# lixirui142/VidToMe

Measured on AMD Instinct MI355X. Metric: denoising steps/sec, 16-frame 512x512 SD-1.5 chunk, ratio=0.5, higher is better.
Workload: dtype f16 tokens; matching f16-MFMA filter + f32 exact refine (f32-identical indices); attention f16 MFMA with f32 accumulate

## Files before the change

### include/vidtome_hip.h

```cpp
#ifndef VIDTOME_HIP_H
#define VIDTOME_HIP_H

#include <stddef.h>
#include <stdint.h>

#ifdef __cplusplus
extern "C" {
#endif

#define VTM_ABI_VERSION 2

enum vtm_dtype { VTM_F32 = 0, VTM_F16 = 1, VTM_BF16 = 2 };

enum vtm_status {
    VTM_OK = 0,
    VTM_EINVAL = -1,
    VTM_ELAUNCH = -2,
    VTM_EWORKSPACE = -3
};

typedef void *vtm_stream_t;

int vtm_version(void);
const char *vtm_last_error(void);
// ... 12 lines not shown
              int64_t Nd_pad, int64_t C_pad, int align, uint64_t *best, vtm_stream_t stream);

size_t vtm_match_filtered_ws_bytes(int64_t B, int64_t C, int64_t Ns, int64_t Nd, int align);
int vtm_match_filtered(const void *x0, int64_t P0, const void *x1, int64_t P1, int dtype, int64_t B,
                       int64_t C, const int32_t *a_rows, int64_t Ns, const int32_t *b_rows, int64_t Nd,
                       int align, void *ws, size_t ws_bytes, uint64_t *best, int32_t *flags_out,
                       vtm_stream_t stream);
int vtm_match_filtered_seeded(const void *x0, int64_t P0, const void *x1, int64_t P1, int dtype, int64_t B,
                              int64_t C, const int32_t *a_rows, int64_t Ns, const int32_t *b_rows, int64_t Nd,
                              int align, void *ws, size_t ws_bytes, uint64_t *best, int32_t *flags_out,
                              int64_t seed_L, int64_t seed_N, const int32_t *seed_pos1, const int32_t *seed_table,
                              vtm_stream_t stream);
#define VTM_MATCH_ONE_LAUNCH 0
#define VTM_MATCH_SCOUT_RANGE 1
#define VTM_MATCH_SCOUT_STEPS(k) (((k) & 0xff) << 8)
int vtm_match_filtered_plan(const void *x0, int64_t P0, const void *x1, int64_t P1, int dtype, int64_t B,
                            int64_t C, const int32_t *a_rows, int64_t Ns, const int32_t *b_rows, int64_t Nd,
                            int align, void *ws, size_t ws_bytes, uint64_t *best, int32_t *flags_out,
                            int64_t seed_L, int64_t seed_N, const int32_t *seed_pos1, const int32_t *seed_table,
                            int mode, vtm_stream_t stream);

#define VTM_POSITION_ORDER_MAX_N 16360
size_t vtm_position_order_counter_ints(int64_t B, int64_t N);
size_t vtm_position_order_ws_bytes(int64_t B, int64_t Ns, int64_t Nd, int64_t N);
int vtm_position_order(const int32_t *a_rows, int64_t Ns, const int32_t *b_rows, int64_t Nd, int64_t B, int64_t L,
                       int64_t N, const int32_t *pos1, int64_t P0, int64_t P1, int32_t *counters, void *ws,
                       size_t ws_bytes, int32_t *a_sorted, int32_t *a_order, int32_t *b_sorted, int32_t *b_order,
                       int32_t *table, int shared_order, vtm_stream_t stream);
int vtm_match_filtered_ordered(const void *x0, int64_t P0, const void *x1, int64_t P1, int dtype, int64_t B,
                               int64_t C, const int32_t *a_sorted, int64_t Ns, const int32_t *b_sorted, int64_t Nd,
                               int align, void *ws, size_t ws_bytes, uint64_t *best, int32_t *flags_out, int64_t seed_L,
                               int64_t seed_N, const int32_t *seed_pos1, const int32_t *seed_table, int mode,
                               const int32_t *a_order, const int32_t *b_order, vtm_stream_t stream);

int vtm_decode_best(const uint64_t *best, int64_t n, float *node_max, int32_t *node_idx,
// ... 158 lines not shown
```

### vidtome_amd/_lib.py

```python
from __future__ import annotations

import ctypes
import functools
import os
import threading
from typing import Optional, Tuple

import torch

_HERE = os.path.dirname(os.path.abspath(__file__))
ABI_VERSION = 2
LIB_PATH = os.environ.get("VIDTOME_HIP_LIB") or os.path.join(_HERE, "lib", "libvidtome_hip.so")

VTM_F32, VTM_F16, VTM_BF16 = 0, 1, 2
ROW_PAD, K_PAD = 256, 32

_DT = {torch.float32: VTM_F32, torch.float16: VTM_F16, torch.bfloat16: VTM_BF16}

_vp, _i64, _int, _f32 = ctypes.c_void_p, ctypes.c_int64, ctypes.c_int, ctypes.c_float
_lib: Optional[ctypes.CDLL] = None

_SIGNATURES = {
    "vtm_version": ([], _int),
    "vtm_last_error": ([], ctypes.c_char_p),
    "vtm_build_ablations": ([], _int),
    "vtm_pad_rows": ([_i64], _i64),
    "vtm_pad_k": ([_i64], _i64),
    "vtm_normalize_gather": ([_vp, _i64, _vp, _i64, _int, _i64, _i64, _vp, _i64, _vp, _vp, _i64, _i64, _vp], _int),
    "vtm_match": ([_vp, _vp, _i64, _i64, _i64, _i64, _i64, _i64, _int, _vp, _vp], _int),
    "vtm_match_filtered_ws_bytes": ([_i64, _i64, _i64, _i64, _int], ctypes.c_size_t),
    "vtm_match_filtered": ([_vp, _i64, _vp, _i64, _int, _i64, _i64, _vp, _i64, _vp, _i64, _int, _vp, ctypes.c_size_t,
                            _vp, _vp, _vp], _int),
    "vtm_match_filtered_plan": ([_vp, _i64, _vp, _i64, _int, _i64, _i64, _vp, _i64, _vp, _i64, _int, _vp, ctypes.c_size_t,
                                 _vp, _vp, _i64, _i64, _vp, _vp, _int, _vp], _int),
    "vtm_match_filtered_ordered": ([_vp, _i64, _vp, _i64, _int, _i64, _i64, _vp, _i64, _vp, _i64, _int, _vp, ctypes.c_size_t,
                                    _vp, _vp, _i64, _i64, _vp, _vp, _int, _vp, _vp, _vp], _int),
    "vtm_position_order_counter_ints": ([_i64, _i64], ctypes.c_size_t),
    "vtm_position_order_ws_bytes": ([_i64, _i64, _i64, _i64], ctypes.c_size_t),
    "vtm_position_order": ([_vp, _i64, _vp, _i64, _i64, _i64, _i64, _vp, _i64, _i64, _vp, _vp, ctypes.c_size_t, _vp, _vp, _vp,
                            _vp, _vp, _int, _vp], _int),
    "vtm_match_filtered_seeded": ([_vp, _i64, _vp, _i64, _int, _i64, _i64, _vp, _i64, _vp, _i64, _int, _vp, ctypes.c_size_t,
                                   _vp, _vp, _i64, _i64, _vp, _vp, _vp], _int),
    "vtm_anchor_pos": ([_vp, _i64, _i64, _i64, _i64, _vp, _i64, _vp, _vp], _int),
    "vtm_decode_best": ([_vp, _i64, _vp, _vp, _vp], _int),
    "vtm_sort_ws_bytes": ([_i64, _i64], ctypes.c_size_t),
    "vtm_sort_desc": ([_vp, _i64, _i64, _vp, _vp, ctypes.c_size_t, _vp], _int),
    "vtm_partition_counts": ([_i64, _i64, _i64, _i64, _i64, ctypes.POINTER(_i64), ctypes.POINTER(_i64)], _int),
    "vtm_partition_local": ([_vp, _i64, _i64, _i64, _i64, _i64, _i64, _vp, _vp, _vp, _vp, _i64, _i64, _vp], _int),
    "vtm_partition_global": ([_vp, _i64, _i64, _i64, _i64, _int, _vp, _vp, _vp, _vp, _vp, _i64, _vp, _vp], _int),
    "vtm_plan_apply": ([_vp, _vp, _vp, _vp, _vp, _vp, _i64, _i64, _i64, _i64, _i64, _int, _vp, _vp, _vp, _vp,
                        _vp, _vp], _int),
# ... 163 lines not shown
                                      _ptr(norms), _ptr(out), n_pad, C_pad, _stream()), "vtm_normalize_gather")
    return out, norms


@_on_device
def match(a: torch.Tensor, b: torch.Tensor, Ns: int, Nd: int, align: bool) -> torch.Tensor:
    B, G, _, Ns_pad, _ = a.shape
    C_pad, Nd_pad = G * 8, b.shape[3]
    best = torch.empty((1 if align else B, Ns), dtype=torch.int64, device=a.device)
    _check(lib().vtm_match(_ptr(a), _ptr(b), B, Ns, Nd, Ns_pad, Nd_pad, C_pad, int(align), _ptr(best), _stream()),
           "vtm_match")
    return best


MATCH_ONE_LAUNCH, MATCH_SCOUT_RANGE = 0, 1


@_on_device
def match_filtered(x0: torch.Tensor, x1: Optional[torch.Tensor], a_rows: torch.Tensor, b_rows: torch.Tensor,
                   align: bool, want_flag: bool = False, seed=None, mode: int = MATCH_ONE_LAUNCH,
                   stats_host: Optional[torch.Tensor] = None, order=None, scout_steps: int = 0):
    _req(x0, "x0"), _req(a_rows, "a_rows"), _req(b_rows, "b_rows")
    B, P0, C = x0.shape
    P1 = 0 if x1 is None else _req(x1, "x1").shape[1]
    Ns, Nd = a_rows.shape[1], b_rows.shape[1]
    nbytes = lib().vtm_match_filtered_ws_bytes(B, C, Ns, Nd, int(align))
    ws = _workspace("match", nbytes, x0.device)
    best = torch.empty((1 if align else B, Ns), dtype=torch.int64, device=x0.device)
    flag = torch.zeros((8,), dtype=torch.int32, device=x0.device) if want_flag else None
    flags_out = _ptr(flag)
    if flag is None and stats_host is not None:
        if not (stats_host.is_pinned() and stats_host.dtype == torch.int32 and stats_host.numel() >= 8):
            raise RuntimeError("match_filtered: stats_host must be a pinned int32 tensor of 8 elements")
        flags_out = stats_host.data_ptr()
    mode = int(mode) | ((int(scout_steps) & 0xff) << 8)
    sN = sL = 0
    pos1 = table = None
    if seed is not None and SEED_MATCHER:
        sN, sL, pos1, table = seed
        if pos1 is not None and (pos1.dtype != torch.int32 or tuple(pos1.shape) != (B, P1) or not pos1.is_contiguous()):
            raise RuntimeError("match_filtered: seed positions must be a contiguous (B, P1) int32 tensor")
        if table is not None and (table.dtype != torch.int32 or tuple(table.shape) != (B, sN) or not table.is_contiguous()):
            raise RuntimeError("match_filtered: the seed table must be a contiguous (B, N) int32 tensor")
    if order is not None:
        a_order, b_order = order
        for o, n, name in ((a_order, Ns, "a_order"), (b_order, Nd, "b_order")):
            if o.dtype != torch.int32 or tuple(o.shape) != (B, n) or not o.is_contiguous() or not o.is_cuda:
                raise RuntimeError(f"match_filtered: {name} must be a contiguous (B, {n}) int32 device tensor")
        _check(lib().vtm_match_filtered_ordered(_ptr(x0), P0, _ptr(x1), P1, dtype_code(x0), B, C, _ptr(a_rows), Ns,
                                                _ptr(b_rows), Nd, int(align), _ptr(ws), nbytes, _ptr(best), flags_out, int(sL), int(sN),
                                                _ptr(pos1), _ptr(table), int(mode), _ptr(a_order), _ptr(b_order), _stream()),
               "vtm_match_filtered_ordered")
        return (best, flag) if want_flag else best
    _check(lib().vtm_match_filtered_plan(_ptr(x0), P0, _ptr(x1), P1, dtype_code(x0), B, C, _ptr(a_rows), Ns,
                                         _ptr(b_rows), Nd, int(align), _ptr(ws), nbytes, _ptr(best), flags_out,
                                         int(sL), int(sN), _ptr(pos1), _ptr(table), int(mode), _stream()),
           "vtm_match_filtered_plan")
    return (best, flag) if want_flag else best


POSITION_ORDER_MAX_N = 16360
_ZEROED: dict = {}


def _zeroed_counters(n_ints: int, device: torch.device) -> torch.Tensor:
    key = (device.index, torch.cuda.current_stream(device).cuda_stream, threading.get_ident())
    buf = _ZEROED.get(key)
    if buf is None or buf.numel() < n_ints:
        buf = torch.zeros((max(int(n_ints), 16),), dtype=torch.int32, device=device)
        with _WS_LOCK:
            _ZEROED[key] = buf
    return buf

# ... 715 lines not shown
```

### vidtome_amd/csrc/match_filter.hip

```cpp
#include "common.h"
#include "ablate.h"
#include "match_plan.h"

#include <algorithm>
#include <type_traits>

namespace {

using namespace vtm_match_plan;
static_assert(MODE_SCOUT_RANGE == VTM_MATCH_SCOUT_RANGE, "match_plan.h restates the public mode value");
constexpr int THREADS = 256;
constexpr float SCALE = 1024.0f;
constexpr float INV_S2 = 1.0f / (1024.0f * 1024.0f);
constexpr float WINDOW = SRC_LO ? 6.5e-4f : DST_LO ? 1.5e-3f : 2.4e-3f;
constexpr int MAX_C = 1280;

typedef float f32x16 __attribute__((ext_vector_type(16)));
typedef _Float16 h16x8 __attribute__((ext_vector_type(8)));
typedef uint32_t u32x4 __attribute__((ext_vector_type(4)));
typedef __attribute__((address_space(3))) void lds_void;
typedef const __attribute__((address_space(1))) void glb_void;

using vtm::to_f32;

template <typename T>
// ... 693 lines not shown
        if (s == s && __builtin_fabsf(s) <= 1.5f && acc_ok && !dry) {
            atomicMax(&amax[align ? i : b * Ns + i], orderable(s));
            atomicMax(&seed_lb[align ? i : b * Ns + i], orderable(s0 - lb_margin));
        }
    }
}

static_assert(RROWS == 32 || RROWS == 64 || RROWS == 128 || RROWS == 256, "refine rows per workgroup");
template <typename T>
__global__ __launch_bounds__(256) void refine_kernel(const T *__restrict__ x0, int64_t P0, const T *__restrict__ x1,
                                                     int64_t P1, int64_t B, int64_t C,
                                                     const int32_t *__restrict__ a_rows, int64_t Ns,
                                                     const int32_t *__restrict__ b_rows, int64_t Nd,
                                                     const float *__restrict__ na, const float *__restrict__ nb,
                                                     int align, int *__restrict__ flags, int64_t rows_out,
                                                     const unsigned int *__restrict__ amax, const int *__restrict__ cnt,
                                                     const uint2 *__restrict__ cand, int *__restrict__ ovf_cnt,
                                                     int *__restrict__ ovf_rows, uint2 *__restrict__ pairs,
                                                     const float *__restrict__ tile_rest, int64_t n_tile_rest,
                                                     unsigned long long *__restrict__ best,
                                                     const int32_t *__restrict__ src_order,
                                                     const int32_t *__restrict__ dst_order) {
    __shared__ int wave_tot[4];
    __shared__ int s_base;
    const int tid = threadIdx.x, lane = tid & 63, wave = tid >> 6;
    {
        bool bad = false;
        for (int64_t t = tid; t < n_tile_rest; t += 256) bad |= !(tile_rest[t] < INFINITY);
        if (__syncthreads_or(bad)) {
            if (blockIdx.x == 0 && tid == 0) {
                flags[0] = 1;
                flags[1] = 1;
            }
            return;
        }
    }
    const int64_t row = (int64_t)blockIdx.x * RROWS + tid;
// ... 24 lines not shown
        unsigned long long todo = __ballot(ovf);
        while (todo) {
            const int lead = __ffsll(todo) - 1;
            const int l0 = __shfl(l, lead, 64);
            const unsigned long long grp = __ballot(ovf && l == l0);
            int base = 0;
            if (lane == lead) {
                base = atomicAdd(&ovf_cnt[l0], __popcll(grp));
                atomicAdd(&flags[2], __popcll(grp));
            }
            base = __shfl(base, lead, 64);
            if (ovf && l == l0)
                ovf_rows[(int64_t)l0 * Ns + base + __popcll(grp & ((1ull << lane) - 1ull))] = (int)(row - (int64_t)l0 * Ns);
            todo &= ~grp;
        }
    }
    int incl = ns;
#pragma unroll
    for (int off = 1; off < 64; off <<= 1) {
        const int t = __shfl_up(incl, off, 64);
        if (lane >= off) incl += t;
    }
    if (lane == 63) wave_tot[wave] = incl;
    __syncthreads();
    int before = 0, total = 0;
#pragma unroll
    for (int w = 0; w < 4; ++w) {
        before += w < wave ? wave_tot[w] : 0;
        total += wave_tot[w];
    }
// ... 64 lines not shown
constexpr int XPD = XD + 1, XPS = XS + 1;
constexpr int XSB = XS / 128;
constexpr int XSU = XS / 64;
static_assert(XS == 128 || XS == 256, "src tile");

__device__ __forceinline__ int64_t xcdiv(int64_t a, int64_t b) { return (a + b - 1) / b; }

template <typename T, bool ORD>
__global__ __launch_bounds__(256, XS == 128 ? 2 : 1) void exact_rows_kernel(
    const T *__restrict__ x0, int64_t P0, const T *__restrict__ x1, int64_t P1, int64_t B, int64_t C,
    const int32_t *__restrict__ a_rows, int64_t Ns, const int32_t *__restrict__ b_rows, int64_t Nd,
    const float *__restrict__ na, const float *__restrict__ nb, int align, const int *__restrict__ flags,
    const int *__restrict__ ovf_cnt, const int *__restrict__ ovf_rows, unsigned long long *__restrict__ best, int nsplit,
    int tiles_per_split, const float *__restrict__ rest_a, const float *__restrict__ rest_bt, int KX, int64_t Ns_pad,
    int64_t rest_tiles, const unsigned int *__restrict__ seed_lb, int *__restrict__ work,
    const int32_t *__restrict__ src_order, const int32_t *__restrict__ dst_order, int32_t *__restrict__ flags_pub) {
    if (flags_pub != nullptr && blockIdx.x == 0 && threadIdx.x < 8) flags_pub[threadIdx.x] = flags[threadIdx.x];
    __shared__ __attribute__((aligned(16))) float sD[8 * XPD * 4];
    __shared__ uint32_t sOrd[ORD ? 2 : 1][ORD ? XD : 1];
    __shared__ __attribute__((aligned(16))) float sS[8 * XPS * 4];
    constexpr int RAW = sizeof(T) == 4 ? 2 : 1;

    const int tid = threadIdx.x, lane = tid & 63;
    const int wave = __builtin_amdgcn_readfirstlane(tid >> 6);
    const int l31 = lane & 31, kh = lane >> 5;
    const bool all = flags[0] != 0;
    const int64_t nlists = align ? 1 : B, nsel = align ? B : 1;
    const int KT = (int)xcdiv(C, XK);
    const int nd_tiles = (int)xcdiv(Nd, XD);
    const int prow = tid >> 2, pg = tid & 3;

    __shared__ int64_t s_item;
    for (int64_t item = blockIdx.x;;) {
        int64_t rem = item, l = 0, cnt_l = 0;
        for (; l < nlists; ++l) {
            cnt_l = all ? Ns : (int64_t)ovf_cnt[l];
            const int64_t items_l = xcdiv(cnt_l, XS) * nsel * nsplit;
            if (rem < items_l) break;
            rem -= items_l;
        }
        if (l == nlists) break;
        const int split = (int)(rem % nsplit);
        rem /= nsplit;
        const int64_t bi = align ? rem % nsel : l;
        const int64_t tile = rem / nsel;
        const int jt0 = split * tiles_per_split, jt1 = min(jt0 + tiles_per_split, nd_tiles);
        auto next_item = [&]() {
            __syncthreads();
            if (tid == 0) s_item = (int64_t)gridDim.x + atomicAdd(work, 1);
            __syncthreads();
            return s_item;
        };
        if (jt0 >= jt1) {
            item = next_item();
            continue;
        }
        auto listed = [&](int r) -> int64_t {
            const int64_t at = tile * XS + r;
            if (at >= cnt_l) return -1;
            return all ? at : (int64_t)ovf_rows[l * Ns + at];
        };

        const T *ps[XSU];
        RowDivisor ds[XSU];
        bool vs[XSU];
#pragma unroll
        for (int u = 0; u < XSU; ++u) {
            const int64_t i = listed(prow + 64 * u);
            vs[u] = i >= 0;
            const int64_t ii = vs[u] ? i : 0;
            ps[u] = pool_row(x0, P0, x1, P1, bi, a_rows[bi * Ns + ii], C);
            ds[u] = row_divisor(na[bi * Ns + ii]);
        }
        const T *pd[2];
        RowDivisor dd[2];
        bool vd[2];
        auto dst_rows = [&](int jt) {
#pragma unroll
            for (int u = 0; u < 2; ++u) {
                const int64_t j = (int64_t)jt * XD + prow + 64 * u;
                vd[u] = j < Nd;
                const int64_t jj = vd[u] ? j : 0;
                pd[u] = pool_row(x0, P0, x1, P1, bi, b_rows[bi * Nd + jj], C);
                dd[u] = row_divisor(nb[bi * Nd + jj]);
                if constexpr (ORD)
                    if (pg == 0) sOrd[jt & 1][prow + 64 * u] = vd[u] ? (uint32_t)dst_order[bi * Nd + jj] : 0xffffffffu;
            }
        };
        uint4 raw[2 + XSU][RAW];
        auto fetch = [&](int kt) {
            const int64_t k = (int64_t)kt * XK + pg * 8;
            const bool kin = k < C;
#pragma unroll
            for (int h = 0; h < RAW; ++h) {
#pragma unroll
                for (int u = 0; u < 2; ++u)
                    raw[u][h] = (kin && vd[u]) ? *reinterpret_cast<const uint4 *>(pd[u] + k + h * (8 / RAW)) : make_uint4(0, 0, 0, 0);
#pragma unroll
                for (int u = 0; u < XSU; ++u)
                    raw[2 + u][h] = (kin && vs[u]) ? *reinterpret_cast<const uint4 *>(ps[u] + k + h * (8 / RAW)) : make_uint4(0, 0, 0, 0);
            }
// ... 24 lines not shown
#pragma unroll
                    for (int j = 0; j < 8; ++j) o[j] = div_by_row(f[j], d);
                } else {
#pragma unroll
                    for (int j = 0; j < 8; ++j) o[j] = f[j] / d.n;
                }
            }
            *reinterpret_cast<float4 *>(&panel[((pg * 2 + 0) * XP + row) * 4]) = make_float4(o[0], o[2], o[4], o[6]);
            *reinterpret_cast<float4 *>(&panel[((pg * 2 + 1) * XP + row) * 4]) = make_float4(o[1], o[3], o[5], o[7]);
        };

        f32x16 acc[4][XSB];
        float bestv[XSB];
        uint32_t besti[XSB];
        float floor_[XSB], rest_l[XSB];
        const bool can_prune = !all && rest_a != nullptr && KX > 0 && KX < KT;
#pragma unroll
        for (int sb = 0; sb < XSB; ++sb) {
            bestv[sb] = -INFINITY;
            besti[sb] = 0xffffffffu;
            const int64_t i = listed(wave * (32 * XSB) + sb * 32 + l31);
            floor_[sb] = (can_prune && i >= 0) ? from_orderable(seed_lb[align ? i : l * Ns + i]) : -INFINITY;
            rest_l[sb] = (can_prune && i >= 0) ? rest_a[bi * Ns_pad + i] : 0.0f;
            if (i < 0) floor_[sb] = INFINITY;
        }
        dst_rows(jt0);
        fetch(0);
        int kt = 0, jt = jt0;
        while (jt < jt1) {
            __syncthreads();
#pragma unroll
            for (int u = 0; u < 2; ++u) stage(raw[u], dd[u], vd[u], sD, XPD, prow + 64 * u);
#pragma unroll
            for (int u = 0; u < XSU; ++u) stage(raw[2 + u], ds[u], vs[u], sS, XPS, prow + 64 * u);
            __syncthreads();
            const bool wrap = kt + 1 == KT;
            if (!wrap || jt + 1 < jt1) {
                if (wrap) dst_rows(jt + 1);
                fetch(wrap ? 0 : kt + 1);
            }
#pragma unroll
            for (int g = 0; g < 4; ++g) {
                float4 af[4];
#pragma unroll
                for (int ib = 0; ib < 4; ++ib) af[ib] = *reinterpret_cast<const float4 *>(&sD[((g * 2 + kh) * XPD + ib * 32 + l31) * 4]);
                float bv[XSB][4];
#pragma unroll
                for (int sb = 0; sb < XSB; ++sb) {
                    const float4 bf = *reinterpret_cast<const float4 *>(&sS[((g * 2 + kh) * XPS + wave * (32 * XSB) + sb * 32 + l31) * 4]);
                    bv[sb][0] = bf.x; bv[sb][1] = bf.y; bv[sb][2] = bf.z; bv[sb][3] = bf.w;
                }
#pragma unroll
                for (int e = 0; e < 4; ++e) {
#pragma unroll
                    for (int ib = 0; ib < 4; ++ib) {
                        const float av = e == 0 ? af[ib].x : e == 1 ? af[ib].y : e == 2 ? af[ib].z : af[ib].w;
#pragma unroll
                        for (int sb = 0; sb < XSB; ++sb) {
                            f32x16 c = acc[ib][sb];
                            if (kt == 0 && g == 0 && e == 0) {
#pragma unroll
                                for (int r = 0; r < 16; ++r) c[r] = 0.0f;
                            }
                            acc[ib][sb] = __builtin_amdgcn_mfma_f32_32x32x2f32(av, bv[sb][e], c, 0, 0, 0);
                        }
                    }
                }
            }
            if (wrap) {
                const int dst0 = jt * XD + 4 * kh;
                const bool full = (int64_t)(jt + 1) * XD <= Nd;
#pragma unroll
                for (int sb = 0; sb < XSB; ++sb) {
                    float bv_ = bestv[sb];
                    uint32_t bi_ = besti[sb];
#pragma unroll
                    for (int ib = 0; ib < 4; ++ib) {
#pragma unroll
                        for (int r = 0; r < 16; ++r) {
                            const int d = dst0 + ib * 32 + (r & 3) + 8 * (r >> 2);
                            const float sc = acc[ib][sb][r];
                            bool upd = !(sc <= bv_) && (bv_ == bv_);
                            uint32_t od = (uint32_t)d;
                            if constexpr (ORD) {
                                od = sOrd[jt & 1][d - jt * XD];
                                upd = upd || (((sc == bv_) || (sc != sc && bv_ != bv_)) && od < bi_);
                            }
                            if (!full) upd = upd && (d < Nd);
                            bv_ = upd ? sc : bv_;
                            bi_ = upd ? od : bi_;
                        }
                    }
                    bestv[sb] = bv_;
                    besti[sb] = bi_;
                }
                ++jt;
                kt = 0;
            } else if (can_prune && kt + 1 == KX) {
                const float rb = rest_bt[bi * rest_tiles + jt] * (1.0f + 0x1p-9f) * INV_S2;
                bool dead = true;
#pragma unroll
                for (int sb = 0; sb < XSB; ++sb) {
                    float pm = -INFINITY;
#pragma unroll
                    for (int ib = 0; ib < 4; ++ib)
#pragma unroll
                        for (int r = 0; r < 16; ++r) pm = fmaxf(pm, acc[ib][sb][r]);
                    dead = dead && (pm + rest_l[sb] * rb + 1e-4f < fmaxf(bestv[sb], floor_[sb]));
                }
                if (__syncthreads_and(dead)) {
                    ++jt;
                    kt = 0;
                    if (jt < jt1) {
                        dst_rows(jt);
                        fetch(0);
                    }
                } else {
                    ++kt;
                }
            } else {
                ++kt;
            }
        }
#pragma unroll
        for (int sb = 0; sb < XSB; ++sb) {
            const int64_t i = listed(wave * (32 * XSB) + sb * 32 + l31);
            if (i >= 0 && besti[sb] != 0xffffffffu) {
                const uint32_t col = besti[sb] + (align ? (uint32_t)(bi * Nd) : 0u);
                const int64_t orow = align ? (ORD ? (int64_t)src_order[i] : i) : l * Ns + (ORD ? (int64_t)src_order[l * Ns + i] : i);
                atomicMax(&best[orow], ((unsigned long long)orderable(bestv[sb]) << 32) | (uint32_t)(~col));
            }
        }
        item = next_item();
    }
}

struct Workspace {
    float *na, *nb;
    uint4 *ah, *al, *bh, *bl;
    unsigned int *amax, *seedlb, *tilemap;
    int *cnt, *flags, *ovf_rows, *ovf_cnt;
    uint2 *cand, *pairs;
    float *rest_a, *rest_bt, *rest_a2, *rest_bt2;
    int64_t zero_words;

    Workspace(void *ws, const Layout &L) : zero_words((int64_t)((L.cand - L.amax) / 4)) {
// ... 16 lines not shown
}

VTM_EXPORT size_t vtm_match_filtered_ws_bytes(int64_t B, int64_t C, int64_t Ns, int64_t Nd, int align) {
    if (B <= 0 || C <= 0 || Ns <= 0 || Nd <= 0) return 0;
    return make_layout(B, C, Ns, Nd, align).total;
}

static int match_filtered_impl(const void *x0, int64_t P0, const void *x1, int64_t P1, int dtype, int64_t B,
                               int64_t C, const int32_t *a_rows, int64_t Ns, const int32_t *b_rows, int64_t Nd,
                               int align, void *ws, size_t ws_bytes, uint64_t *best, int32_t *flags_out,
                               int64_t seed_L, int64_t seed_N, const int32_t *seed_pos1, const int32_t *seed_table,
                               int mode, const int32_t *src_order, const int32_t *dst_order, vtm_stream_t stream) {
    const char *what = "vtm_match_filtered";
    VTM_REQUIRE(x0 && a_rows && b_rows && ws && best, "vtm_match_filtered: null pointer");
    const int scout_steps = (mode >> 8) & 0xff;
    mode &= 0xff;
    VTM_REQUIRE((src_order == nullptr) == (dst_order == nullptr), "vtm_match_filtered_ordered: both inverse maps or none");
    VTM_REQUIRE(mode == VTM_MATCH_ONE_LAUNCH || mode == VTM_MATCH_SCOUT_RANGE, "vtm_match_filtered: bad mode %d", mode);
    VTM_REQUIRE(B > 0 && C > 0 && C % 8 == 0 && Ns > 0 && Nd > 0, "vtm_match_filtered: bad sizes");
    VTM_REQUIRE(P1 == 0 || x1, "vtm_match_filtered: x1 is null but P1 > 0");
    VTM_REQUIRE(B * Nd < (1ll << 32) - 1, "vtm_match_filtered: index space overflow");
    VTM_REQUIRE(C <= MAX_C, "vtm_match_filtered: C=%lld > %d (error window derived for C <= %d; use vtm_match)",
                (long long)C, MAX_C, MAX_C);
    const Layout L = make_layout(B, C, Ns, Nd, align);
    if (ws_bytes < L.total)
        return vtm::fail(VTM_EWORKSPACE, "vtm_match_filtered: workspace %zu < %zu bytes", ws_bytes, L.total);
    const int64_t rows_out = align ? Ns : B * Ns;
    VTM_REQUIRE(rows_out * CAP < (1ll << 31), "vtm_match_filtered: too many rows for the 32-bit candidate index");
    VTM_REQUIRE(dtype == VTM_F32 || dtype == VTM_F16 || dtype == VTM_BF16, "vtm_match_filtered: bad dtype");

// ... 28 lines not shown
                      unsigned int *tilemap) {
        hipLaunchKernelGGL(kernel, dim3((unsigned)grid), dim3(THREADS), 0, s, W.ah, W.al, W.bh, W.bl, Ns, Nd, L.Ns_pad, L.Nd_pad,
                           L.C64, align, P.ns_tiles, P.nd_tiles, nsplit, tps, P.total_src_tiles, P.patch_tiles, W.amax, W.cnt, W.cand,
                           (int)rows_out, W.flags, rest_a, rest_bt, kp, flags_out != nullptr ? 1 : 0, tilemap, P.map_words);
    };
    if (P.range_plan) {
        filter(filter_kernel<true>, P.grid, P.nsplit, P.tiles_per_split, shallow ? W.rest_a2 : W.rest_a,
               shallow ? W.rest_bt2 : W.rest_bt, P.KPS, W.tilemap);
        filter(filter_kernel<false>, P.grid_r, P.nsplit_r, P.tps_r, W.rest_a, W.rest_bt, P.KP, W.tilemap);
    } else {
        filter(filter_kernel<false>, P.grid, P.nsplit, P.tiles_per_split, P.prune ? W.rest_a : nullptr,
               P.prune ? W.rest_bt : nullptr, P.prune ? P.KP : 0x7fffffff, nullptr);
    }

    int32_t *flags_pub = kernel_writable(flags_out);
    vtm::with_dtype(dtype, what, [&](auto t) {
        using T = decltype(t);
        hipLaunchKernelGGL(refine_kernel<T>, dim3(P.refine_grid), block, 0, s, (const T *)x0, P0, (const T *)x1, P1, B, C, a_rows, Ns,
                           b_rows, Nd, W.na, W.nb, align, W.flags, rows_out, W.amax, W.cnt, W.cand, W.ovf_cnt, W.ovf_rows, W.pairs,
                           (const float *)W.rest_bt, B * (L.Nd_pad / FBD), bp, src_order, dst_order);
        hipLaunchKernelGGL((src_order ? exact_rows_kernel<T, true> : exact_rows_kernel<T, false>), dim3(P.xgrid), block, 0, s,
                           (const T *)x0, P0, (const T *)x1, P1, B, C, a_rows, Ns, b_rows, Nd, W.na, W.nb, align, W.flags, W.ovf_cnt,
                           W.ovf_rows, bp, P.xsplit, P.xtps, (const float *)W.rest_a, (const float *)W.rest_bt, P.KX, L.Ns_pad,
                           L.Nd_pad / FBD, (const unsigned int *)W.seedlb, W.flags + 6, src_order, dst_order, flags_pub);
        return VTM_OK;
    });
    if (int rc = vtm::launch_status(what)) return rc;

    if (flags_out && !flags_pub) {
        const hipError_t e = hipMemcpyAsync(flags_out, W.flags, 8 * sizeof(int), hipMemcpyDefault, s);
        if (e != hipSuccess) return vtm::fail(VTM_ELAUNCH, "vtm_match_filtered: copy: %s", hipGetErrorString(e));
    }
    return VTM_OK;
}

VTM_EXPORT int vtm_match_filtered(const void *x0, int64_t P0, const void *x1, int64_t P1, int dtype, int64_t B,
                                  int64_t C, const int32_t *a_rows, int64_t Ns, const int32_t *b_rows, int64_t Nd,
                                  int align, void *ws, size_t ws_bytes, uint64_t *best, int32_t *flags_out,
                                  vtm_stream_t stream) {
    return match_filtered_impl(x0, P0, x1, P1, dtype, B, C, a_rows, Ns, b_rows, Nd, align, ws, ws_bytes, best, flags_out, 0, 0,
                               nullptr, nullptr, VTM_MATCH_ONE_LAUNCH, nullptr, nullptr, stream);
}

VTM_EXPORT int vtm_match_filtered_seeded(const void *x0, int64_t P0, const void *x1, int64_t P1, int dtype, int64_t B,
                                         int64_t C, const int32_t *a_rows, int64_t Ns, const int32_t *b_rows, int64_t Nd,
                                         int align, void *ws, size_t ws_bytes, uint64_t *best, int32_t *flags_out,
                                         int64_t seed_L, int64_t seed_N, const int32_t *seed_pos1, const int32_t *seed_table,
                                         vtm_stream_t stream) {
    VTM_REQUIRE(seed_N >= 0 && seed_L >= 0, "vtm_match_filtered_seeded: bad seed description");
// ... 29 lines not shown
```

### vidtome_amd/csrc/match_plan.h

```cpp
#pragma once
#include <cstddef>
#include <cstdint>
#include <cstdlib>

namespace vtm_match_plan {

constexpr int FBD = 128;
constexpr int FBS = 256;
constexpr int FBK = 64;
constexpr int CAP = 64;
#ifndef VTM_FILTER_PRODUCTS
#define VTM_FILTER_PRODUCTS 1
#endif
constexpr bool SRC_LO = VTM_FILTER_PRODUCTS >= 3;
constexpr bool DST_LO = VTM_FILTER_PRODUCTS >= 2;
static_assert(DST_LO || !SRC_LO, "the src lo half is only used together with the dst lo half");
#ifndef VTM_PREP_WAVES
#define VTM_PREP_WAVES 4
#endif
constexpr int PREP_WAVES = VTM_PREP_WAVES;
#ifndef VTM_RROWS
#define VTM_RROWS 64
#endif
constexpr int RROWS = VTM_RROWS;
#ifndef VTM_XS
#define VTM_XS 128
#endif
constexpr int XS = VTM_XS;
constexpr int XD = 128;
constexpr int XK = 32;
constexpr int MODE_SCOUT_RANGE = 1;

inline int64_t cdiv(int64_t a, int64_t b) { return (a + b - 1) / b; }
inline size_t align_up(size_t v) { return (v + 255) & ~(size_t)255; }

struct Layout {
    size_t na, nb, ah, al, bh, bl, amax, cnt, seedlb, tilemap, cand, flags, ovf_cnt, ovf, pairs, rest_a, rest_bt, rest_a2, rest_bt2, total;
    int64_t Ns_pad, Nd_pad, C64;
};

inline Layout make_layout(int64_t B, int64_t C, int64_t Ns, int64_t Nd, int align) {
    Layout L;
    L.Ns_pad = cdiv(Ns, FBS) * FBS;
    L.Nd_pad = cdiv(Nd, FBS) * FBS;
    L.C64 = cdiv(C, 64) * 64;
    const int64_t rows_out = align ? Ns : B * Ns;
// ... 13 lines not shown
    L.ovf_cnt = take((size_t)B * 4);
    L.cand = take((size_t)rows_out * CAP * 8);
    L.ovf = take((size_t)rows_out * 4);
    L.pairs = take((size_t)rows_out * CAP * 8);
    L.rest_a = take((size_t)B * L.Ns_pad * 4);
    L.rest_bt = take((size_t)B * (L.Nd_pad / FBD) * 4);
    L.rest_a2 = take((size_t)B * L.Ns_pad * 4);
    L.rest_bt2 = take((size_t)B * (L.Nd_pad / FBD) * 4);
    L.total = o;
    return L;
}

struct DebugEnv {
    int kp5, kp, nsplit;
    bool seed_dry, nsplit_r4, no_xprune;
};
inline const DebugEnv &debug_env() {
    static const DebugEnv e = [] {
        auto num = [](const char *name) {
            const char *v = getenv(name);
            return v ? atoi(v) : -1;
        };
        DebugEnv d;
        d.kp5 = num("VTM_DEBUG_KP5");
        d.kp = num("VTM_DEBUG_KP");
        d.nsplit = num("VTM_DEBUG_NSPLIT");
        d.seed_dry = getenv("VTM_DEBUG_SEED_DRY") != nullptr;
        d.nsplit_r4 = getenv("VTM_DEBUG_NSPLIT_R4") != nullptr;
        d.no_xprune = getenv("VTM_DEBUG_NOXPRUNE") != nullptr;
        return d;
    }();
    return e;
}

struct FilterPlan {
    int KT, KP, KPS;
    bool prune;
    int64_t cut, cut2;
    int ns_tiles, nd_tiles, total_src_tiles, patch_tiles, ngroups;
    int nsplit, tiles_per_split;
    int64_t grid;
    bool range_plan;
    int tps_r, nsplit_r;
    int64_t grid_r;
// ... 92 lines not shown
```

Before: 22.37.

## Add banded exact-rows pass for warps whose candidate columns cluster in a narrow range

```diff
diff --git a/include/vidtome_hip.h b/include/vidtome_hip.h
--- a/include/vidtome_hip.h
+++ b/include/vidtome_hip.h
@@ -50,11 +50,15 @@
 #define VTM_MATCH_ONE_LAUNCH 0
 #define VTM_MATCH_SCOUT_RANGE 1
 #define VTM_MATCH_SCOUT_STEPS(k) (((k) & 0xff) << 8)
+#define VTM_MATCH_NO_BAND (1 << 16)
 int vtm_match_filtered_plan(const void *x0, int64_t P0, const void *x1, int64_t P1, int dtype, int64_t B,
                             int64_t C, const int32_t *a_rows, int64_t Ns, const int32_t *b_rows, int64_t Nd,
                             int align, void *ws, size_t ws_bytes, uint64_t *best, int32_t *flags_out,
                             int64_t seed_L, int64_t seed_N, const int32_t *seed_pos1, const int32_t *seed_table,
                             int mode, vtm_stream_t stream);
+int vtm_match_filtered_band_stats(const void *ws, int64_t B, int64_t C, int64_t Ns, int64_t Nd, int align, int32_t *out,
+                                  vtm_stream_t stream);
+int vtm_match_band_pays(int blocks, int pairs, int64_t C);
 
 #define VTM_POSITION_ORDER_MAX_N 16360
 size_t vtm_position_order_counter_ints(int64_t B, int64_t N);
diff --git a/vidtome_amd/_lib.py b/vidtome_amd/_lib.py
--- a/vidtome_amd/_lib.py
+++ b/vidtome_amd/_lib.py
@@ -35,6 +35,8 @@
                                  _vp, _vp, _i64, _i64, _vp, _vp, _int, _vp], _int),
     "vtm_match_filtered_ordered": ([_vp, _i64, _vp, _i64, _int, _i64, _i64, _vp, _i64, _vp, _i64, _int, _vp, ctypes.c_size_t,
                                     _vp, _vp, _i64, _i64, _vp, _vp, _int, _vp, _vp, _vp], _int),
+    "vtm_match_filtered_band_stats": ([_vp, _i64, _i64, _i64, _i64, _int, _vp, _vp], _int),
+    "vtm_match_band_pays": ([_int, _int, _i64], _int),
     "vtm_position_order_counter_ints": ([_i64, _i64], ctypes.c_size_t),
     "vtm_position_order_ws_bytes": ([_i64, _i64, _i64, _i64], ctypes.c_size_t),
     "vtm_position_order": ([_vp, _i64, _vp, _i64, _i64, _i64, _i64, _vp, _i64, _i64, _vp, _vp, ctypes.c_size_t, _vp, _vp, _vp,
@@ -228,12 +230,13 @@
 
 
 MATCH_ONE_LAUNCH, MATCH_SCOUT_RANGE = 0, 1
+MATCH_NO_BAND = 1 << 16
 
 
 @_on_device
 def match_filtered(x0: torch.Tensor, x1: Optional[torch.Tensor], a_rows: torch.Tensor, b_rows: torch.Tensor,
                    align: bool, want_flag: bool = False, seed=None, mode: int = MATCH_ONE_LAUNCH,
-                   stats_host: Optional[torch.Tensor] = None, order=None, scout_steps: int = 0):
+                   stats_host: Optional[torch.Tensor] = None, order=None, scout_steps: int = 0, band: bool = True):
     _req(x0, "x0"), _req(a_rows, "a_rows"), _req(b_rows, "b_rows")
     B, P0, C = x0.shape
     P1 = 0 if x1 is None else _req(x1, "x1").shape[1]
@@ -247,7 +250,7 @@
         if not (stats_host.is_pinned() and stats_host.dtype == torch.int32 and stats_host.numel() >= 8):
             raise RuntimeError("match_filtered: stats_host must be a pinned int32 tensor of 8 elements")
         flags_out = stats_host.data_ptr()
-    mode = int(mode) | ((int(scout_steps) & 0xff) << 8)
+    mode = int(mode) | ((int(scout_steps) & 0xff) << 8) | (0 if band else MATCH_NO_BAND)
     sN = sL = 0
     pos1 = table = None
     if seed is not None and SEED_MATCHER:
@@ -271,6 +274,23 @@
                                          int(sL), int(sN), _ptr(pos1), _ptr(table), int(mode), _stream()),
            "vtm_match_filtered_plan")
     return (best, flag) if want_flag else best
+
+
+def match_band_stats(x0: torch.Tensor, a_rows: torch.Tensor, b_rows: torch.Tensor, align: bool):
+    B, _, C = x0.shape
+    Ns, Nd = a_rows.shape[1], b_rows.shape[1]
+    nbytes = lib().vtm_match_filtered_ws_bytes(B, C, Ns, Nd, int(align))
+    ws = _workspace("match", nbytes, x0.device)
+    out = torch.zeros((2,), dtype=torch.int32, device=x0.device)
+    with torch.cuda.device(x0.device):
+        _check(lib().vtm_match_filtered_band_stats(_ptr(ws), B, C, Ns, Nd, int(align), _ptr(out), _stream()),
+               "vtm_match_filtered_band_stats")
+    blocks, rows = out.tolist()
+    return blocks, rows
+
+
+def match_band_pays(blocks: int, pairs: int, C: int) -> bool:
+    return bool(lib().vtm_match_band_pays(int(blocks), int(pairs), int(C)))
 
 
 POSITION_ORDER_MAX_N = 16360
diff --git a/vidtome_amd/csrc/match_filter.hip b/vidtome_amd/csrc/match_filter.hip
--- a/vidtome_amd/csrc/match_filter.hip
+++ b/vidtome_amd/csrc/match_filter.hip
@@ -9,6 +9,7 @@
 
 using namespace vtm_match_plan;
 static_assert(MODE_SCOUT_RANGE == VTM_MATCH_SCOUT_RANGE, "match_plan.h restates the public mode value");
+static_assert(MODE_NO_BAND == VTM_MATCH_NO_BAND, "match_plan.h restates the public mode bit");
 constexpr int THREADS = 256;
 constexpr float SCALE = 1024.0f;
 constexpr float INV_S2 = 1.0f / (1024.0f * 1024.0f);
@@ -732,13 +733,13 @@
                                                      const int32_t *__restrict__ b_rows, int64_t Nd,
                                                      const float *__restrict__ na, const float *__restrict__ nb,
                                                      int align, int *__restrict__ flags, int64_t rows_out,
-                                                     const unsigned int *__restrict__ amax, const int *__restrict__ cnt,
+                                                     const unsigned int *__restrict__ amax, int *__restrict__ cnt,
                                                      const uint2 *__restrict__ cand, int *__restrict__ ovf_cnt,
                                                      int *__restrict__ ovf_rows, uint2 *__restrict__ pairs,
                                                      const float *__restrict__ tile_rest, int64_t n_tile_rest,
                                                      unsigned long long *__restrict__ best,
                                                      const int32_t *__restrict__ src_order,
-                                                     const int32_t *__restrict__ dst_order) {
+                                                     const int32_t *__restrict__ dst_order, int band_k) {
     __shared__ int wave_tot[4];
     __shared__ int s_base;
     const int tid = threadIdx.x, lane = tid & 63, wave = tid >> 6;
@@ -793,6 +794,45 @@
                 ovf_rows[(int64_t)l0 * Ns + base + __popcll(grp & ((1ull << lane) - 1ull))] = (int)(row - (int64_t)l0 * Ns);
             todo &= ~grp;
         }
+    }
+    if (band_k > 0) {
+        const bool on = live && !ovf && ns > 0;
+        int lo = 0x7fffffff, hi = -1;
+        if (on) {
+#pragma unroll
+            for (int c = 0; c < PRE; ++c)
+                if (__uint_as_float(pre[c].x) >= thr) {
+                    lo = min(lo, (int)pre[c].y);
+                    hi = max(hi, (int)pre[c].y);
+                }
+            for (int c = PRE; c < n; ++c) {
+                const uint2 cd = cand[(int64_t)c * rows_out + row];
+                if (__uint_as_float(cd.x) >= thr) {
+                    lo = min(lo, (int)cd.y);
+                    hi = max(hi, (int)cd.y);
+                }
+            }
+        }
+        int bp = on ? ns : 0;
+#pragma unroll
+        for (int off = 16; off > 0; off >>= 1) {
+            lo = min(lo, __shfl_xor(lo, off, 64));
+            hi = max(hi, __shfl_xor(hi, off, 64));
+            bp += __shfl_xor(bp, off, 64);
+        }
+        const uint32_t mask = (uint32_t)(__ballot(on) >> (lane & 32));
+        const int64_t row0 = row - (lane & 31), rowl = min(row0 + 31, rows_out - 1);
+        const bool slot = tid < RROWS && row0 + BAND_REC_INTS <= rows_out;
+        const bool take = slot && hi >= 0 && row0 / Ns == rowl / Ns && band_pays(hi / 32 - lo / 32 + 1, bp, C, band_k);
+        if (slot && (lane & 31) == 0) {
+            *reinterpret_cast<int4 *>(cnt + row0) = take ? make_int4(lo, hi, (int)mask, bp) : make_int4(0, -1, 0, 0);
+            if (take) {
+                atomicAdd(&flags[BAND_FLAGS], 1);
+                atomicAdd(&flags[BAND_FLAGS + 1], __popc(mask));
+                atomicAdd(&flags[3], bp);
+            }
+        }
+        if (take) ns = 0;
     }
     int incl = ns;
 #pragma unroll
@@ -887,7 +927,8 @@
     const int *__restrict__ ovf_cnt, const int *__restrict__ ovf_rows, unsigned long long *__restrict__ best, int nsplit,
     int tiles_per_split, const float *__restrict__ rest_a, const float *__restrict__ rest_bt, int KX, int64_t Ns_pad,
     int64_t rest_tiles, const unsigned int *__restrict__ seed_lb, int *__restrict__ work,
-    const int32_t *__restrict__ src_order, const int32_t *__restrict__ dst_order, int32_t *__restrict__ flags_pub) {
+    const int32_t *__restrict__ src_order, const int32_t *__restrict__ dst_order, int32_t *__restrict__ flags_pub,
+    const int *__restrict__ band_rec, int64_t rows_out) {
     if (flags_pub != nullptr && blockIdx.x == 0 && threadIdx.x < 8) flags_pub[threadIdx.x] = flags[threadIdx.x];
     __shared__ __attribute__((aligned(16))) float sD[8 * XPD * 4];
     __shared__ uint32_t sOrd[ORD ? 2 : 1][ORD ? XD : 1];
@@ -903,6 +944,9 @@
     const int nd_tiles = (int)xcdiv(Nd, XD);
     const int prow = tid >> 2, pg = tid & 3;
 
+    static_assert(BAND_REC_INTS == 4, "a band record is one int4");
+    const int64_t band_items = (XS == 128 && band_rec != nullptr && flags[BAND_FLAGS] > 0) ? xcdiv(rows_out, XS) : 0;
+    int64_t bpass = -1;
     __shared__ int64_t s_item;
     for (int64_t item = blockIdx.x;;) {
         int64_t rem = item, l = 0, cnt_l = 0;
@@ -912,26 +956,87 @@
             if (rem < items_l) break;
             rem -= items_l;
         }
-        if (l == nlists) break;
-        const int split = (int)(rem % nsplit);
-        rem /= nsplit;
-        const int64_t bi = align ? rem % nsel : l;
-        const int64_t tile = rem / nsel;
-        const int jt0 = split * tiles_per_split, jt1 = min(jt0 + tiles_per_split, nd_tiles);
+        const bool band = l == nlists;
+        if (band && rem >= band_items) break;
         auto next_item = [&]() {
             __syncthreads();
             if (tid == 0) s_item = (int64_t)gridDim.x + atomicAdd(work, 1);
             __syncthreads();
             return s_item;
         };
+        int64_t bi, tile;
+        int jt0, jt1;
+        int blo[4], bhi[4];
+        uint32_t bmask[4];
+        if (!band) {
+            const int split = (int)(rem % nsplit);
+            rem /= nsplit;
+            bi = align ? rem % nsel : l;
+            tile = rem / nsel;
+            jt0 = split * tiles_per_split, jt1 = min(jt0 + tiles_per_split, nd_tiles);
+#pragma unroll
+            for (int q = 0; q < 4; ++q) blo[q] = 0, bhi[q] = 0x7fffffff, bmask[q] = 0xffffffffu;
+        } else {
+            tile = rem;
+            int64_t next = -1;
+#pragma unroll
+            for (int q = 0; q < 4; ++q) {
+                const int64_t r0 = tile * XS + 32 * q;
+                const int4 rc = r0 + BAND_REC_INTS <= rows_out ? *reinterpret_cast<const int4 *>(band_rec + r0) : make_int4(0, -1, 0, 0);
+                blo[q] = rc.x, bhi[q] = rc.y, bmask[q] = (uint32_t)rc.z;
+                const int64_t smp = r0 / Ns;
+                if (bmask[q] != 0u && smp > bpass && (next < 0 || smp < next)) next = smp;
+            }
+            if (next < 0) {
+                bpass = -1;
+                item = next_item();
+                continue;
+            }
+            bi = l = next;
+            jt0 = 0x7fffffff, jt1 = 0;
+#pragma unroll
+            for (int q = 0; q < 4; ++q) {
+                if (bmask[q] == 0u || (tile * XS + 32 * q) / Ns != bi || blo[q] < 0 || bhi[q] >= Nd || blo[q] > bhi[q])
+                    bmask[q] = 0u, blo[q] = 0x7fffffff, bhi[q] = -1;
+                if (bmask[q] != 0u) jt0 = min(jt0, blo[q] / XD), jt1 = max(jt1, bhi[q] / XD + 1);
+            }
+        }
         if (jt0 >= jt1) {
+            if (band) {
+                bpass = bi;
+                continue;
+            }
             item = next_item();
             continue;
         }
         auto listed = [&](int r) -> int64_t {
             const int64_t at = tile * XS + r;
+            if (band) {
+                const int q = r >> 5;
+                const uint32_t m = q == 0 ? bmask[0] : q == 1 ? bmask[1] : q == 2 ? bmask[2] : bmask[3];
+                return ((m >> (r & 31)) & 1u) ? at - bi * Ns : -1;
+            }
             if (at >= cnt_l) return -1;
             return all ? at : (int64_t)ovf_rows[l * Ns + at];
+        };
+        auto advance = [&](int t) {
+            if (band)
+                for (; t < jt1; ++t) {
+                    bool need = false;
+#pragma unroll
+                    for (int q = 0; q < 4; ++q) need |= blo[q] / XD <= t && t <= bhi[q] / XD;
+                    if (need) break;
+                }
+            return t;
+        };
+        const int wq = XS == 128 ? wave : 0;
+        const int wlo = __builtin_amdgcn_readfirstlane((wq == 0 ? blo[0] : wq == 1 ? blo[1] : wq == 2 ? blo[2] : blo[3]) / 32);
+        const int whi = __builtin_amdgcn_readfirstlane((wq == 0 ? bhi[0] : wq == 1 ? bhi[1] : wq == 2 ? bhi[2] : bhi[3]) / 32);
+        auto blocks_of = [&](int t) {
+            int m = 0;
+#pragma unroll
+            for (int ib = 0; ib < 4; ++ib) m |= (t * 4 + ib >= wlo && t * 4 + ib <= whi) ? 1 << ib : 0;
+            return m;
         };
 
         const T *ps[XSU];
@@ -948,7 +1053,7 @@
         const T *pd[2];
         RowDivisor dd[2];
         bool vd[2];
-        auto dst_rows = [&](int jt) {
+        auto dst_rows = [&](int jt, int buf) {
 #pragma unroll
             for (int u = 0; u < 2; ++u) {
                 const int64_t j = (int64_t)jt * XD + prow + 64 * u;
@@ -957,7 +1062,7 @@
                 pd[u] = pool_row(x0, P0, x1, P1, bi, b_rows[bi * Nd + jj], C);
                 dd[u] = row_divisor(nb[bi * Nd + jj]);
                 if constexpr (ORD)
-                    if (pg == 0) sOrd[jt & 1][prow + 64 * u] = vd[u] ? (uint32_t)dst_order[bi * Nd + jj] : 0xffffffffu;
+                    if (pg == 0) sOrd[buf][prow + 64 * u] = vd[u] ? (uint32_t)dst_order[bi * Nd + jj] : 0xffffffffu;
             }
         };
         uint4 raw[2 + XSU][RAW];
@@ -1012,7 +1117,7 @@
         float bestv[XSB];
         uint32_t besti[XSB];
         float floor_[XSB], rest_l[XSB];
-        const bool can_prune = !all && rest_a != nullptr && KX > 0 && KX < KT;
+        const bool can_prune = !all && !band && rest_a != nullptr && KX > 0 && KX < KT;
 #pragma unroll
         for (int sb = 0; sb < XSB; ++sb) {
             bestv[sb] = -INFINITY;
@@ -1022,9 +1127,10 @@
             rest_l[sb] = (can_prune && i >= 0) ? rest_a[bi * Ns_pad + i] : 0.0f;
             if (i < 0) floor_[sb] = INFINITY;
         }
-        dst_rows(jt0);
+        dst_rows(jt0, 0);
         fetch(0);
-        int kt = 0, jt = jt0;
+        int kt = 0, jt = jt0, ob = 0;
+        int ibm = blocks_of(jt0);
         while (jt < jt1) {
             __syncthreads();
 #pragma unroll
@@ -1033,8 +1139,9 @@
             for (int u = 0; u < XSU; ++u) stage(raw[2 + u], ds[u], vs[u], sS, XPS, prow + 64 * u);
             __syncthreads();
             const bool wrap = kt + 1 == KT;
-            if (!wrap || jt + 1 < jt1) {
-                if (wrap) dst_rows(jt + 1);
+            const int nxt = wrap ? advance(jt + 1) : jt;
+            if (!wrap || nxt < jt1) {
+                if (wrap) dst_rows(nxt, ob ^ 1);
                 fetch(wrap ? 0 : kt + 1);
             }
 #pragma unroll
@@ -1052,6 +1159,7 @@
                 for (int e = 0; e < 4; ++e) {
 #pragma unroll
                     for (int ib = 0; ib < 4; ++ib) {
+                        if (!((ibm >> ib) & 1)) continue;
                         const float av = e == 0 ? af[ib].x : e == 1 ? af[ib].y : e == 2 ? af[ib].z : af[ib].w;
 #pragma unroll
                         for (int sb = 0; sb < XSB; ++sb) {
@@ -1074,6 +1182,7 @@
                     uint32_t bi_ = besti[sb];
 #pragma unroll
                     for (int ib = 0; ib < 4; ++ib) {
+                        if (!((ibm >> ib) & 1)) continue;
 #pragma unroll
                         for (int r = 0; r < 16; ++r) {
                             const int d = dst0 + ib * 32 + (r & 3) + 8 * (r >> 2);
@@ -1081,7 +1190,7 @@
                             bool upd = !(sc <= bv_) && (bv_ == bv_);
                             uint32_t od = (uint32_t)d;
                             if constexpr (ORD) {
-                                od = sOrd[jt & 1][d - jt * XD];
+                                od = sOrd[ob][d - jt * XD];
                                 upd = upd || (((sc == bv_) || (sc != sc && bv_ != bv_)) && od < bi_);
                             }
                             if (!full) upd = upd && (d < Nd);
@@ -1092,7 +1201,9 @@
                     bestv[sb] = bv_;
                     besti[sb] = bi_;
                 }
-                ++jt;
+                jt = nxt;
+                ob ^= 1;
+                ibm = blocks_of(jt);
                 kt = 0;
             } else if (can_prune && kt + 1 == KX) {
                 const float rb = rest_bt[bi * rest_tiles + jt] * (1.0f + 0x1p-9f) * INV_S2;
@@ -1108,9 +1219,10 @@
                 }
                 if (__syncthreads_and(dead)) {
                     ++jt;
+                    ob ^= 1;
                     kt = 0;
                     if (jt < jt1) {
-                        dst_rows(jt);
+                        dst_rows(jt, ob);
                         fetch(0);
                     }
                 } else {
@@ -1128,6 +1240,11 @@
                 const int64_t orow = align ? (ORD ? (int64_t)src_order[i] : i) : l * Ns + (ORD ? (int64_t)src_order[l * Ns + i] : i);
                 atomicMax(&best[orow], ((unsigned long long)orderable(bestv[sb]) << 32) | (uint32_t)(~col));
             }
+        }
+        if (band) {
+            bpass = bi;
+            __syncthreads();
+            continue;
         }
         item = next_item();
     }
@@ -1174,6 +1291,7 @@
     const char *what = "vtm_match_filtered";
     VTM_REQUIRE(x0 && a_rows && b_rows && ws && best, "vtm_match_filtered: null pointer");
     const int scout_steps = (mode >> 8) & 0xff;
+    const bool no_band = (mode & VTM_MATCH_NO_BAND) != 0;
     mode &= 0xff;
     VTM_REQUIRE((src_order == nullptr) == (dst_order == nullptr), "vtm_match_filtered_ordered: both inverse maps or none");
     VTM_REQUIRE(mode == VTM_MATCH_ONE_LAUNCH || mode == VTM_MATCH_SCOUT_RANGE, "vtm_match_filtered: bad mode %d", mode);
@@ -1232,15 +1350,17 @@
     }
 
     int32_t *flags_pub = kernel_writable(flags_out);
+    const int band_k = (align || no_band || XS != 128) ? 0 : dbg.band_k >= 0 ? dbg.band_k : BAND_PAIRS_PER_BLOCK;
     vtm::with_dtype(dtype, what, [&](auto t) {
         using T = decltype(t);
         hipLaunchKernelGGL(refine_kernel<T>, dim3(P.refine_grid), block, 0, s, (const T *)x0, P0, (const T *)x1, P1, B, C, a_rows, Ns,
                            b_rows, Nd, W.na, W.nb, align, W.flags, rows_out, W.amax, W.cnt, W.cand, W.ovf_cnt, W.ovf_rows, W.pairs,
-                           (const float *)W.rest_bt, B * (L.Nd_pad / FBD), bp, src_order, dst_order);
+                           (const float *)W.rest_bt, B * (L.Nd_pad / FBD), bp, src_order, dst_order, band_k);
         hipLaunchKernelGGL((src_order ? exact_rows_kernel<T, true> : exact_rows_kernel<T, false>), dim3(P.xgrid), block, 0, s,
                            (const T *)x0, P0, (const T *)x1, P1, B, C, a_rows, Ns, b_rows, Nd, W.na, W.nb, align, W.flags, W.ovf_cnt,
                            W.ovf_rows, bp, P.xsplit, P.xtps, (const float *)W.rest_a, (const float *)W.rest_bt, P.KX, L.Ns_pad,
-                           L.Nd_pad / FBD, (const unsigned int *)W.seedlb, W.flags + 6, src_order, dst_order, flags_pub);
+                           L.Nd_pad / FBD, (const unsigned int *)W.seedlb, W.flags + 6, src_order, dst_order, flags_pub,
+                           band_k > 0 ? (const int *)W.cnt : nullptr, rows_out);
         return VTM_OK;
     });
     if (int rc = vtm::launch_status(what)) return rc;
@@ -1251,6 +1371,19 @@
     }
     return VTM_OK;
 }
+
+VTM_EXPORT int vtm_match_filtered_band_stats(const void *ws, int64_t B, int64_t C, int64_t Ns, int64_t Nd, int align,
+                                             int32_t *out, vtm_stream_t stream) {
+    VTM_REQUIRE(ws && out, "vtm_match_filtered_band_stats: null pointer");
+    VTM_REQUIRE(B > 0 && C > 0 && Ns > 0 && Nd > 0, "vtm_match_filtered_band_stats: bad sizes");
+    const Layout L = make_layout(B, C, Ns, Nd, align);
+    const hipError_t e = hipMemcpyAsync(out, static_cast<const char *>(ws) + L.flags + BAND_FLAGS * sizeof(int), 2 * sizeof(int),
+                                        hipMemcpyDefault, vtm::as_stream(stream));
+    if (e != hipSuccess) return vtm::fail(VTM_ELAUNCH, "vtm_match_filtered_band_stats: copy: %s", hipGetErrorString(e));
+    return VTM_OK;
+}
+
+VTM_EXPORT int vtm_match_band_pays(int blocks, int pairs, int64_t C) { return band_pays(blocks, pairs, C) ? 1 : 0; }
 
 VTM_EXPORT int vtm_match_filtered(const void *x0, int64_t P0, const void *x1, int64_t P1, int dtype, int64_t B,
                                   int64_t C, const int32_t *a_rows, int64_t Ns, const int32_t *b_rows, int64_t Nd,
diff --git a/vidtome_amd/csrc/match_plan.h b/vidtome_amd/csrc/match_plan.h
--- a/vidtome_amd/csrc/match_plan.h
+++ b/vidtome_amd/csrc/match_plan.h
@@ -30,6 +30,21 @@
 constexpr int XD = 128;
 constexpr int XK = 32;
 constexpr int MODE_SCOUT_RANGE = 1;
+constexpr int MODE_NO_BAND = 1 << 16;
+
+constexpr int BAND_FLAGS = 8;
+constexpr int BAND_REC_INTS = 4;
+constexpr int BAND_PAIRS_PER_BLOCK = 32;
+constexpr int64_t BAND_FIXED = 2048;
+#if defined(__HIP__)
+#define VTM_PLAN_HD __host__ __device__
+#else
+#define VTM_PLAN_HD
+#endif
+VTM_PLAN_HD inline bool band_pays(int blocks, int pairs, int64_t C, int k = BAND_PAIRS_PER_BLOCK) {
+    if (blocks <= 0 || pairs <= 0 || C <= 0 || k <= 0) return false;
+    return (int64_t)pairs * C >= (int64_t)blocks * ((int64_t)k * C + BAND_FIXED);
+}
 
 inline int64_t cdiv(int64_t a, int64_t b) { return (a + b - 1) / b; }
 inline size_t align_up(size_t v) { return (v + 255) & ~(size_t)255; }
@@ -73,6 +88,7 @@
 struct DebugEnv {
     int kp5, kp, nsplit;
     bool seed_dry, nsplit_r4, no_xprune;
+    int band_k = -1;
 };
 inline const DebugEnv &debug_env() {
     static const DebugEnv e = [] {
@@ -87,6 +103,7 @@
         d.seed_dry = getenv("VTM_DEBUG_SEED_DRY") != nullptr;
         d.nsplit_r4 = getenv("VTM_DEBUG_NSPLIT_R4") != nullptr;
         d.no_xprune = getenv("VTM_DEBUG_NOXPRUNE") != nullptr;
+        d.band_k = num("VTM_DEBUG_BAND_K");
         return d;
     }();
     return e;
```

Result: slower. 21.33 (-4.7%).
